# Mikata-Project/adcraft

Hardware: AMD Instinct MI355X
Metric: env-steps/sec (envs×keywords auctions/s) (higher is better)
Workload: dtype i32 cents + f32 (Philox4x32-7 u32); 1 GPU; cfg2: 4096 envs x 256 keywords per GPU, IMPLICIT keywords, mean_volume 128, cvr 0.8, no_vol_prob 0.0, drift False, budget non-binding, 60-step episodes with auto-reset; envs_per_gpu=4096, keywords=256, parallelism=env-sharded x1, collective=none (single GPU), weak_scaling_reference=also.cfg4.value of the N=1 --full line (same per-GPU shard as the N>1 runs)

## Files before the change

adcraft_amd/csrc/adc_law.h:

```cpp
#pragma once
#include <stdint.h>

#if defined(__HIPCC__)
#include <hip/hip_runtime.h>
#define ADC_HD __host__ __device__ __forceinline__
#else
#include <math.h>
#define ADC_HD static inline
#endif

namespace adc {

enum Stage : uint32_t { ST_VOL = 0, ST_AUCTION = 1, ST_DRIFT = 2, ST_XPHANTOM = 3, ST_XREV = 4, ST_ACTION = 5, ST_METRIC = 6, ST_CONV = 7, ST_KEYGEN = 8, ST_AGENT = 9,
                        ST_GBIDDERS = 10, ST_GBID = 11, ST_GCLICK = 12, ST_INTERP = 13, ST_MLP = 14 };
constexpr int kTimesteps = 24;
constexpr int kVolumeMax = 1 << 20;
constexpr float kMoneyMaxCents = 1.0e9f;

struct U4 { uint32_t x, y, z, w; };

ADC_HD uint32_t xor3(uint32_t a, uint32_t b, uint32_t c)
{
#if defined(__HIP_DEVICE_COMPILE__)
    return __builtin_amdgcn_bitop3_b32(a, b, c, 0x96);
// ... 557 lines not shown
    if (any_lane(bound_open(t))) return lower_bound_finish(t, target, loc, scale, tab, stage);
    return bound_accepted(t);
}

ADC_HD uint32_t lower_bound_v(int32_t target, float loc, float scale, const LogTableEntry *tab)
{
    int stage;
    return lower_bound_v_staged(target, loc, scale, tab, stage);
}

ADC_HD void lower_bound_pair(int32_t bid_c, float loc, float scale, const LogTableEntry *tab, uint32_t &w_lo, uint32_t &w_hi, int &stage)
{
    const int32_t b_lo = lower_bound_window(1 - bid_c, loc, scale, tab), b_hi = lower_bound_window(bid_c, loc, scale, tab);
    const BoundTrial t_lo = bound_trial(b_lo, 1 - bid_c, loc, scale, tab), t_hi = bound_trial(b_hi, bid_c, loc, scale, tab);
    w_lo = bound_accepted(t_lo);
    w_hi = bound_accepted(t_hi);
    stage = kBoundAccepted;
    if (any_lane(bound_open(t_lo) || bound_open(t_hi))) {
        int s_lo = kBoundAccepted, s_hi = kBoundAccepted;
        w_lo = lower_bound_finish(t_lo, 1 - bid_c, loc, scale, tab, s_lo);
        w_hi = lower_bound_finish(t_hi, bid_c, loc, scale, tab, s_hi);
        stage = s_lo > s_hi ? s_lo : s_hi;
    }
}

ADC_HD uint64_t offset_reaching_f64(uint32_t W, uint32_t m, uint64_t range)
{
    if (W == 0u) return 0ull;
    if (W > 0x00FFFFFFu || m == 0u) return range;
    const double q = ((double)W * 4294967296.0) / (double)m;
    if (!(q < (double)range)) return range;
    uint64_t d = (uint64_t)q;
    const uint64_t need = (uint64_t)W << 32;
    if (d * m >= need) { if (d > 0ull && (d - 1ull) * m >= need) d -= 1ull; }
    else { d += 1ull; if (d * m < need) d += 1ull; }
    return d < range ? d : range;
}

enum OffsetPath : int { kOffsetCandidate = 0, kOffsetF64 = 1 };

struct OffsetDivisor { uint32_t m; float inv, inv4096; uint64_t m2, m3; };

ADC_HD OffsetDivisor offset_divisor(uint32_t m)
{
    const float inv = fast_rcp((float)m);
    return OffsetDivisor{m, inv, inv * 4096.0f, 2ull * m, 3ull * m};
}

struct OffsetTrial { uint32_t d; bool ok; };

ADC_HD OffsetTrial offset_trial(uint32_t W, const OffsetDivisor &v)
{
    const uint32_t d0 = to_word((float)W * 4294967296.0f * v.inv);
    const uint64_t need = (uint64_t)W << 32;
    const int64_t r0 = (int64_t)(need - (uint64_t)d0 * v.m);
    const uint32_t d1 = d0 + (uint32_t)to_int(__builtin_ceilf((float)(int32_t)(r0 >> 12) * v.inv4096));
    const uint64_t u = need + v.m2 - (uint64_t)d1 * v.m;
    const uint32_t d = d1 - 1u + (u > (uint64_t)v.m ? 1u : 0u) + (u > v.m2 ? 1u : 0u);
    const bool none = W > 0x00FFFFFFu;
    OffsetTrial t;
    t.ok = none | (((u - 1ull) < v.m3) & (v.m >= 0x01000000u));
    t.d = none ? 0xFFFFFFFFu : d;
    return t;
}

ADC_HD uint64_t offset_reaching_staged(uint32_t W, uint32_t m, uint64_t range, int &path)
{
    const OffsetTrial t = offset_trial(W, offset_divisor(m));
    uint64_t d = (W > 0x00FFFFFFu || !((uint64_t)t.d < range)) ? range : (uint64_t)t.d;
    path = kOffsetCandidate;
    if (any_lane(!t.ok)) {
        if (!t.ok) { d = offset_reaching_f64(W, m, range); path = kOffsetF64; }
    }
    return d;
}

ADC_HD uint64_t offset_reaching(uint32_t W, uint32_t m, uint64_t range)
{
    int path;
    return offset_reaching_staged(W, m, range, path);
}

struct WinIntervals { uint32_t c_lo, c_w, n_lo, n_w; };

template <bool F64 = false>
ADC_HD WinIntervals win_intervals_of_bounds(uint32_t w_lo, uint32_t w_hi, uint64_t t_click, const AuctionLaw &law, int *path = nullptr)
{
    WinIntervals r{0u, 0u, 0u, 0u};
    if (path) *path = F64 ? kOffsetF64 : kOffsetCandidate;
    if (!(w_lo < w_hi)) return r;
    const uint64_t top = 0xFFFFFFFFull;
    const uint64_t range_n = 4294967296ull - t_click;
    if constexpr (F64) {
        uint64_t a = offset_reaching_f64(w_lo, law.m_click, t_click), b = offset_reaching_f64(w_hi, law.m_click, t_click);
        b = b < top ? b : top;
        if (a < b) { r.c_lo = (uint32_t)a; r.c_w = (uint32_t)(b - a); }
        a = t_click + offset_reaching_f64(w_lo, law.m_noclick, range_n);
        b = t_click + offset_reaching_f64(w_hi, law.m_noclick, range_n);
        b = b < top ? b : top;
        if (a < b) { r.n_lo = (uint32_t)a; r.n_w = (uint32_t)(b - a); }
    } else {
        const OffsetDivisor vc = offset_divisor(law.m_click), vn = offset_divisor(law.m_noclick);
        const OffsetTrial ta = offset_trial(w_lo, vc), tb = offset_trial(w_hi, vc), tan = offset_trial(w_lo, vn), tbn = offset_trial(w_hi, vn);
        const uint32_t t32 = t_click < top ? (uint32_t)t_click : 0xFFFFFFFFu;
        uint32_t a = ta.d < t32 ? ta.d : t32, b = tb.d < t32 ? tb.d : t32, an = sat_add(t32, tan.d), bn = sat_add(t32, tbn.d);
        const bool all_ok = ta.ok & tb.ok & tan.ok & tbn.ok;
        if (any_lane(!all_ok)) {
#pragma unroll 1
            for (int i = 0; i < 4; ++i) {
                const bool click = i < 2, lower = (i & 1) == 0;
                if (!(i == 0 ? ta.ok : i == 1 ? tb.ok : i == 2 ? tan.ok : tbn.ok)) {
                    uint64_t d = offset_reaching_f64(lower ? w_lo : w_hi, click ? law.m_click : law.m_noclick, click ? t_click : range_n);
                    d += click ? 0ull : t_click;
                    const uint32_t d32 = d < top ? (uint32_t)d : 0xFFFFFFFFu;
                    a = i == 0 ? d32 : a;
                    b = i == 1 ? d32 : b;
                    an = i == 2 ? d32 : an;
                    bn = i == 3 ? d32 : bn;
                }
            }
            if (path && !all_ok) *path = kOffsetF64;
        }
        if (a < b) { r.c_lo = a; r.c_w = b - a; }
        if (an < bn) { r.n_lo = an; r.n_w = bn - an; }
    }
    return r;
}

template <bool SIDE_BY_SIDE = true, bool OFFSETS_F64 = false>
ADC_HD WinIntervals win_intervals(int32_t bid_c, float loc, float scale, uint64_t t_click, const AuctionLaw &law, const LogTableEntry *tab)
{
    uint32_t w_lo, w_hi;
    if constexpr (SIDE_BY_SIDE) {
        int stage;
        lower_bound_pair(bid_c, loc, scale, tab, w_lo, w_hi, stage);
    } else {
        w_lo = lower_bound_v(1 - bid_c, loc, scale, tab);
        w_hi = lower_bound_v(bid_c, loc, scale, tab);
    }
    return win_intervals_of_bounds<OFFSETS_F64>(w_lo, w_hi, t_click, law);
}

struct WinBrackets { WinIntervals out, in; };
constexpr float kWordSlack = 4096.0f;

ADC_HD uint32_t sat_sub(uint32_t a, uint32_t b)
{
#if defined(__clang__)
    return __builtin_elementwise_sub_sat(a, b);
#else
    return a > b ? a - b : 0u;
#endif
}
ADC_HD void lower_bound_estimate(float x_t, float loc, float inv_s, float &est, float &slack)
{
    const float z_t = (x_t - loc) * inv_s;
    const float e_t = __builtin_fabsf(z_t);
    const float mag = min_num(fast_exp2(fma32(e_t, -1.44269504f, 23.0f)), 8388607.0f);
    est = z_t < 0.0f ? mag : 16777215.0f - mag;
    const float rel = fma32(1.0e-6f, fma32(__builtin_fabsf(x_t) + __builtin_fabsf(loc), inv_s, e_t), 2.0e-5f);
    slack = min_num(fma32(mag, rel, 16.0f), 33554432.0f);
}

ADC_HD WinBrackets win_brackets(int32_t bid_c, float loc, float scale, float t_f)
{
    const float inv_s = fast_rcp(__builtin_fabsf(scale));
// ... 351 lines not shown
```

adcraft_amd/csrc/adc_shims.cpp:

```cpp
#include <algorithm>
#include <cmath>
#include <cstdint>
#include <thread>
#include <vector>

#include "../../include/adcraft_engine.h"
#include "adc_law.h"
#include "adc_fast_schedule.h"
#include "adc_interp.h"
#include "adc_mlp.h"
#include "adc_es.h"
#include "adc_pg.h"
#include "adc_pg_kl.h"
#include "adc_pg_shuffle.h"
#include "adc_imitation.h"
#include "adc_td3.h"
#include "adc_sac.h"
#include "adc_pbt.h"
#include "adc_norm.h"
#include "adc_rew_norm.h"
#include "adc_td3_norm.h"
#include "adc_sac_norm.h"
#include "adc_per.h"

// ... 160 lines not shown
    const adc::LogTableEntry *table = host_log_table();
    shim_parallel_for(n, [=](int64_t i0, int64_t i1) {
        for (int64_t i = i0; i < i1; ++i) {
            bool whole = false;
            v_out[i] = adc::lower_bound_v_bisect(target[i], loc[i], scale[i], table, &whole);
            if (whole_range_out) whole_range_out[i] = whole ? 1 : 0;
        }
    });
    return ADC_OK;
}

ADC_EXPORT int adc_win_intervals_host(int64_t n, const int32_t *bid_c, const float *cost_loc, const float *cost_scale, const float *buyside_ctr,
                                      int32_t bisect, uint32_t *out4, uint8_t *stage_out)
{
    if (n < 0 || (n > 0 && (!bid_c || !cost_loc || !cost_scale || !buyside_ctr || !out4))) return ADC_EINVAL;
    const adc::LogTableEntry *table = host_log_table();
    shim_parallel_for(n, [=](int64_t i0, int64_t i1) {
        for (int64_t i = i0; i < i1; ++i) {
            const adc::AuctionLaw law = adc::make_auction_law(buyside_ctr[i]);
            const uint64_t t_click = adc::bernoulli_threshold(buyside_ctr[i]);
            uint32_t w_lo, w_hi;
            int stage = 0;
            if (bisect) {
                bool a = false, b = false;
                w_lo = adc::lower_bound_v_bisect(1 - bid_c[i], cost_loc[i], cost_scale[i], table, &a);
                w_hi = adc::lower_bound_v_bisect(bid_c[i], cost_loc[i], cost_scale[i], table, &b);
                stage = (a || b) ? 1 : 0;
            } else {
                adc::lower_bound_pair(bid_c[i], cost_loc[i], cost_scale[i], table, w_lo, w_hi, stage);
            }
            const adc::WinIntervals r = adc::win_intervals_of_bounds(w_lo, w_hi, t_click, law);
            uint32_t *o = out4 + 4 * i;
            o[0] = r.c_lo; o[1] = r.c_w; o[2] = r.n_lo; o[3] = r.n_w;
            if (stage_out) stage_out[i] = (uint8_t)stage;
        }
    });
    return ADC_OK;
}

ADC_EXPORT int adc_offset_reaching_host(int64_t n, const uint32_t *W, const uint32_t *m, const uint64_t *range, uint64_t *d_out, uint8_t *path_out)
{
    if (n < 0 || (n > 0 && (!W || !m || !range || !d_out))) return ADC_EINVAL;
    shim_parallel_for(n, [=](int64_t i0, int64_t i1) {
        for (int64_t i = i0; i < i1; ++i) {
            int path = 0;
            d_out[i] = adc::offset_reaching_staged(W[i], m[i], range[i], path);
            if (path_out) path_out[i] = (uint8_t)path;
        }
    });
    return ADC_OK;
}

ADC_EXPORT int adc_offset_reaching_f64_host(int64_t n, const uint32_t *W, const uint32_t *m, const uint64_t *range, uint64_t *d_out, uint8_t *path_out)
{
    if (n < 0 || (n > 0 && (!W || !m || !range || !d_out))) return ADC_EINVAL;
    shim_parallel_for(n, [=](int64_t i0, int64_t i1) {
        for (int64_t i = i0; i < i1; ++i) {
            d_out[i] = adc::offset_reaching_f64(W[i], m[i], range[i]);
            if (path_out)
                path_out[i] = W[i] == 0u ? 0 : (W[i] > 0x00FFFFFFu || m[i] == 0u) ? 1
                              : !(((double)W[i] * 4294967296.0) / (double)m[i] < (double)range[i]) ? 2 : 3;
        }
    });
    return ADC_OK;
}

ADC_EXPORT int adc_win_intervals_offsets_host(int64_t n, const int32_t *bid_c, const float *cost_loc, const float *cost_scale, const float *buyside_ctr,
                                              int32_t f64, uint32_t *out4, uint8_t *path_out)
{
    if (n < 0 || (n > 0 && (!bid_c || !cost_loc || !cost_scale || !buyside_ctr || !out4))) return ADC_EINVAL;
    const adc::LogTableEntry *table = host_log_table();
    shim_parallel_for(n, [=](int64_t i0, int64_t i1) {
        for (int64_t i = i0; i < i1; ++i) {
            const adc::AuctionLaw law = adc::make_auction_law(buyside_ctr[i]);
            const uint64_t t_click = adc::bernoulli_threshold(buyside_ctr[i]);
            uint32_t w_lo, w_hi;
            int stage = 0, path = 0;
            adc::lower_bound_pair(bid_c[i], cost_loc[i], cost_scale[i], table, w_lo, w_hi, stage);
            const adc::WinIntervals r = f64 ? adc::win_intervals_of_bounds<true>(w_lo, w_hi, t_click, law, &path)
                                            : adc::win_intervals_of_bounds<false>(w_lo, w_hi, t_click, law, &path);
            uint32_t *o = out4 + 4 * i;
            o[0] = r.c_lo; o[1] = r.c_w; o[2] = r.n_lo; o[3] = r.n_w;
            if (path_out) path_out[i] = (uint8_t)path;
        }
    });
    return ADC_OK;
}

ADC_EXPORT int adc_draw_folded_host(int64_t n, const uint64_t *key, const uint32_t *index, const uint32_t *stage, const uint32_t *keyword,
                                    const uint32_t *tick, uint32_t *plain4, uint32_t *folded4, uint32_t *kw4)
{
    if (n < 0 || (n > 0 && (!key || !index || !stage || !keyword || !tick || !plain4 || !folded4 || !kw4))) return ADC_EINVAL;
    shim_parallel_for(n, [=](int64_t i0, int64_t i1) {
        for (int64_t i = i0; i < i1; ++i) {
            const uint32_t tick_k1 = adc::philox_fold_tick(key[i], tick[i]);
            const adc::U4 a = adc::draw(key[i], index[i], stage[i], keyword[i], tick[i]);
            const adc::U4 b = adc::draw_folded(key[i], index[i], stage[i], keyword[i], tick_k1);
            const adc::U4 c = adc::draw_kw_folded(key[i], index[i], adc::philox_kw_half(stage[i], keyword[i], (uint32_t)key[i]), tick_k1);
            uint32_t *pa = plain4 + 4 * i, *pb = folded4 + 4 * i, *pc = kw4 + 4 * i;
            pa[0] = a.x; pa[1] = a.y; pa[2] = a.z; pa[3] = a.w;
            pb[0] = b.x; pb[1] = b.y; pb[2] = b.z; pb[3] = b.w;
            pc[0] = c.x; pc[1] = c.y; pc[2] = c.z; pc[3] = c.w;
        }
    });
    return ADC_OK;
}

ADC_EXPORT int64_t adc_proven_win_price_host(int64_t n, const int32_t *bid_c, const float *cost_loc, const float *cost_scale, const float *buyside_ctr,
                                             int64_t exhaustive_below, int32_t ends, int32_t samples, uint64_t seed, int64_t *checked, int64_t *first_bad3)
{
    if (n < 0 || (n > 0 && (!bid_c || !cost_loc || !cost_scale || !buyside_ctr)) || ends < 0 || samples < 0) return -1;
    const adc::LogTableEntry *table = host_log_table();
    int64_t bad = 0, count = 0, first[3] = {-1, -1, -1};
    uint64_t s = seed | 1ull;
    auto next = [&]() { s ^= s << 13; s ^= s >> 7; s ^= s << 17; return s; };
    for (int64_t i = 0; i < n; ++i) {
        const float loc = cost_loc[i], scale = cost_scale[i];
        auto check = [&](uint32_t v, int route) {
            ++count;
            if (adc::competitor_cents_of_proven_win(v, loc, scale, table) != adc::competitor_cents_from_v(v, loc, scale, table)) {
                if (first[0] < 0) { first[0] = i; first[1] = (int64_t)v; first[2] = route; }
                ++bad;
            }
        };
        uint32_t w_lo, w_hi;
        int stage = 0;
        adc::lower_bound_pair(bid_c[i], loc, scale, table, w_lo, w_hi, stage);
        if (w_lo < w_hi) {
            const uint32_t width = w_hi - w_lo;
            if ((int64_t)width <= exhaustive_below) {
                for (uint32_t v = w_lo; v < w_hi; ++v) check(v, 0);
            } else {
                for (uint32_t e = 0; e < (uint32_t)ends && e < width; ++e) { check(w_lo + e, 0); check(w_hi - 1u - e, 0); }
                for (int32_t k = 0; k < samples; ++k) check(w_lo + (uint32_t)(next() % width), 0);
            }
        }
        const adc::AuctionLaw law = adc::make_auction_law(buyside_ctr[i]);
        const adc::WinIntervals iv = adc::win_intervals_of_bounds(w_lo, w_hi, adc::bernoulli_threshold(buyside_ctr[i]), law);
        if (iv.c_w != 0u) {
            for (int e = 0; e < 2; ++e) {
                const uint32_t word = e == 0 ? iv.c_lo : iv.c_lo + iv.c_w - 1u;
                const uint32_t v = adc::mulhi32(word, law.m_click);
                check(v < 0x00FFFFFFu ? v : 0x00FFFFFFu, 1);
            }
        }
    }
    if (checked) *checked = count;
    if (first_bad3) { first_bad3[0] = first[0]; first_bad3[1] = first[1]; first_bad3[2] = first[2]; }
    return bad;
}

ADC_EXPORT int64_t adc_fast_schedule_host(const int32_t *vol_k, int32_t tile_kw, int32_t tile_index, int32_t *slots7, int64_t cap, int64_t *totals2,
                                          int32_t *info2)
{
    constexpr int B = adc::kFastTileLanes, WL = adc::kFastWaveLanes, NW = adc::kFastTileWaves;
    if (!vol_k || tile_kw < 1 || tile_kw > B || tile_index < 0 || cap < 0 || (cap > 0 && !slots7)) return ADC_EINVAL;
    int V[B];
    int64_t volume = 0, needed = 0;
    int live = 0;
    for (int t = 0; t < B; ++t) {
        V[t] = t < tile_kw ? vol_k[t] : 0;
        if (V[t] < 0 || V[t] > adc::kVolumeMax) return ADC_EINVAL;
        volume += V[t];
        live += V[t] > 0;
        needed += adc::fast_calls_needed(V[t]);
    }
// ... 1553 lines not shown
```

adcraft_amd/csrc/parts/kernel_fast.inc:

```
constexpr int kQueueCap = 128;
constexpr int kDenseVolumePerKeyword = adc::kDenseVolumePerKeyword;
static_assert(kFastBlock == adc::kFastTileLanes && kWave == adc::kFastWaveLanes, "adc_fast_schedule.h describes this workgroup");

struct alignas(16) KwLawA {
    unsigned int m_click, t_conv;
    float loc, scale;
};
struct alignas(16) KwLawB {
    float mu, sd;
    union {
        struct {
            unsigned int t_click;
            int bid_c;
        } d;
        adc::KwHalf conv;
    };
};
union alignas(16) KwWin {
    adc::WinIntervals iv;
    struct { unsigned int m_noclick, pad0, pad1, pad2; } d;
};

constexpr int kClkShift = 21, kConvShift = 42;
constexpr int kVolBits = 21;
// ... 71 lines not shown
        r.key = v.key[env];
        r.tick = v.tick[env];
        r.drift = v.drift_on && v.drift_pending[env];
        const int hint = v.exact_hint[env];
        r.skip = (hint & ~4) == 2;
        r.emit = LISTS && hint == 1 && v.click_rec != nullptr;
        if (tid < tile_kw && k < v.K && !r.skip) {
            r.vol_mean = param_at(v, ADC_P_VOL_MEAN, env, k);
            r.vol_std = param_at(v, ADC_P_VOL_STD, env, k);
            r.bctr = param_at(v, ADC_P_BCTR, env, k);
            r.sctr = param_at(v, ADC_P_SCTR, env, k);
            r.loc = param_at(v, ADC_P_A, env, k);
            r.scale = param_at(v, ADC_P_B, env, k);
            r.mu = param_at(v, ADC_P_REV_MEAN, env, k);
            r.sd = param_at(v, ADC_P_REV_STD, env, k);
            r.bid = bids[(size_t)env * v.K + k];
        }
        return r;
    };

    const int n_tiles = v.N * tiles;
    const int tile_first = blockIdx.x * tiles_per_wg, tile_last = min(tile_first + tiles_per_wg, n_tiles);
    sh.logtab[tid] = g_log_table[tid];
    for (int i = tid; i <= adc::kNormTableEntries; i += kFastBlock) sh.normtab[i] = g_norm_nodes[i];
    FastRaw next = load_tile(tile_first);

  for (int tile_index = tile_first; tile_index < tile_last; ++tile_index) {
    const FastRaw raw = next;
    if (tile_index + 1 < tile_last) next = load_tile(tile_index + 1);
    if (raw.skip) continue;
    const int env = tile_index / tiles;
    const int tile = tile_index - env * tiles;
    const int k = tile * tile_kw + tid;
    const bool valid = tid < tile_kw && k < v.K;
    const uint64_t key = ((uint64_t)(uint32_t)__builtin_amdgcn_readfirstlane((int)(uint32_t)(raw.key >> 32)) << 32) |
                         (uint32_t)__builtin_amdgcn_readfirstlane((int)(uint32_t)raw.key);
    const uint32_t tick = (uint32_t)__builtin_amdgcn_readfirstlane((int)raw.tick);
    uint32_t tick_k1 = adc::philox_fold_tick(key, tick);
    asm volatile("" : "+s"(tick_k1));
    const uint32_t kw_base = (uint32_t)(tile * tile_kw);
    if (LISTS && raw.emit && tid == 0) v.click_tick[env] = tick + 1u;
    if constexpr (LISTS) { if (raw.emit && !NARROW && tid < adc::kTimesteps) ls.row_count[tid] = 0u; }
    [[maybe_unused]] const unsigned long long t_start = FDBG_T();

    if (tid < (tile_kw + 3) / 4) {
        const adc::U4 w = adc::draw(key, 0u, adc::ST_VOL, (kw_base >> 2) + (uint32_t)tid, tick);
        *reinterpret_cast<uint4 *>(&sh.volw[4 * tid]) = make_uint4(w.x, w.y, w.z, w.w);
    }
    float vol_mean = raw.vol_mean, bctr = raw.bctr, sctr = raw.sctr;
    const float vol_std = raw.vol_std, loc = raw.loc, scale = raw.scale, mu = raw.mu, sd = raw.sd, bid = raw.bid;
    if (valid && raw.drift && drift_keyword(v, env, key, tick - 1u, k, vol_mean, vol_std, bctr, sctr)) {
        param_at(v, ADC_P_VOL_MEAN, env, k) = vol_mean;
        param_at(v, ADC_P_BCTR, env, k) = bctr;
        param_at(v, ADC_P_SCTR, env, k) = sctr;
    }
    sh.a_cnt[tid] = sh.a_cost[tid] = sh.a_rev[tid] = 0ull;
    __syncthreads();
    int V = 0;
    if (valid) {
        float x = adc::fma32(vol_std, normal_tab_nodes(sh.volw[tid], sh.normtab), vol_mean);
        x = x > 0.0f ? x : 0.0f;
        x = x < (float)adc::kVolumeMax ? x : (float)adc::kVolumeMax;
        const float t = __builtin_truncf(x);
        V = (int)t + ((x - t) >= 0.5f ? 1 : 0);
    }
    if constexpr (LISTS) {
        if (raw.emit) {
            const int rows = (int)v.click_row_hint[env], s = V / adc::kTimesteps;
            ls.jcut[tid] = rows >= adc::kTimesteps - 1 ? 0x7FFFFFFF : V - (adc::kTimesteps - 1) * s + rows * s;
            if (tid == 0) ls.price_cut = v.click_price_hint[env];
        }
    }
    {
        const int vsum = wave_sum_i32(V);
        const int live = (int)__popcll(__builtin_amdgcn_ballot_w64(V > 0));
        if (lane == 0) { sh.wave_vol[wv] = vsum; sh.wave_live[wv] = live; }
    }
    __syncthreads();
    int tile_volume = 0, tile_live = 0;
#pragma unroll
    for (int i = 0; i < kFastBlock / kWave; ++i) { tile_volume += sh.wave_vol[i]; tile_live += sh.wave_live[i]; }
    const bool dense = adc::fast_tile_dense(tile_volume, tile_live);
    const int chunk_shift = adc::fast_chunk_shift(tile_volume);
    const int nch = adc::fast_full_items(V, chunk_shift);
    const int ntc = adc::fast_tail_calls(V, chunk_shift);
    const int incl = wave_scan_i32(adc::fast_pack_counts(nch, ntc));
    if (lane == 63) sh.wave_tot[wv] = incl;
    FSLOT_ADD(1, (unsigned long long)adc::fast_calls_needed(V));
    [[maybe_unused]] const unsigned long long t_law = FDBG_T();
    if (V > 0) {
        const uint64_t t_click = adc::bernoulli_threshold(bctr);
        const adc::AuctionLaw law = adc::make_auction_law(bctr);
        const int bid_c = (int)adc::bid_to_cents(bid);
        sh.law_a[tid] = KwLawA{law.m_click, adc::saturate_threshold(adc::bernoulli_threshold(sctr)), loc, scale};
        KwLawB lb;
        lb.mu = mu;
        lb.sd = sd;
        if (dense) {
            lb.conv = adc::philox_kw_half(adc::ST_CONV, kw_base + (uint32_t)tid, (uint32_t)key);
            sh.win[tid].iv = adc::win_intervals(bid_c, loc, scale, t_click, law, sh.logtab);
        } else {
            lb.d.t_click = law.t32;
            lb.d.bid_c = bid_c;
            sh.win[tid].d.m_noclick = law.m_noclick;
        }
        sh.law_b[tid] = lb;
    }
    FDBG_ADD(1, FDBG_T() - t_law);
    __syncthreads();
    int wave_base = 0, total = 0, wave_base2 = 0, total2 = 0;
#pragma unroll
    for (int i = 0; i < kFastBlock / kWave; ++i) {
        const int t = sh.wave_tot[i];
        if (i < wv) { wave_base += adc::fast_packed_items(t); wave_base2 += adc::fast_packed_calls(t); }
        total += adc::fast_packed_items(t);
        total2 += adc::fast_packed_calls(t);
    }
    __syncthreads();
    sh.off[tid] = wave_base + adc::fast_packed_items(incl) - nch;
    {
        const int first_call = wave_base2 + adc::fast_packed_calls(incl) - ntc;
        sh.vol[tid] = V | (first_call << kVolBits);
#pragma unroll
        for (int c = 0; c < adc::kFastTailCallsMax; ++c)
            if (c < ntc) sh.tail_kw[first_call + c] = (unsigned char)tid;
    }
    if (tid == 0) sh.off[kFastBlock] = total;
    __syncthreads();
    [[maybe_unused]] const unsigned long long t_p2 = FDBG_T();
    FDBG_ADD(0, t_p2 - t_start);

    const int wq = __builtin_amdgcn_readfirstlane(wv);
    unsigned int *const qtag = sh.queue.tag[wq];
    unsigned int *const qword = sh.queue.word[wq];
    unsigned int qtail = 0;

    auto resolve_click = [&](bool direct) {
        const uint2 ent = make_uint2(qtag[lane], qword[lane]);
        const unsigned int uu = ent.x >> 24;
        unsigned int acc_off = uu * (unsigned int)sizeof(unsigned long long);
        asm volatile("" : "+v"(acc_off));
        unsigned long long *const acc = (unsigned long long *)((char *)sh.a_cnt + acc_off);
        static_assert(sizeof(KwLawA) == 2 * sizeof(unsigned long long) && sizeof(KwLawB) == sizeof(KwLawA), "law records at twice the accumulators' stride");
        unsigned int law_off;
        asm volatile("v_add_u32 %0, %1, %1" : "=v"(law_off) : "v"(acc_off));
        const KwLawA ka = *(const KwLawA *)((const char *)sh.law_a + law_off);
        const KwLawB kb = *(const KwLawB *)((const char *)sh.law_b + law_off);
        unsigned int price = ent.y;
        if (!direct) {
            unsigned int vv = adc::mulhi32(ent.y, ka.m_click);
            vv = vv < 0x00FFFFFFu ? vv : 0x00FFFFFFu;
            price = (unsigned int)adc::competitor_cents_of_proven_win(vv, ka.loc, ka.scale, sh.logtab);
        }
        const adc::U4 w2 = direct ? adc::draw_folded(key, ent.x & 0x00FFFFFFu, adc::ST_CONV, kw_base + uu, tick_k1)
                                  : adc::draw_kw_folded(key, ent.x & 0x00FFFFFFu, kb.conv, tick_k1);
        const bool conv = adc::bernoulli32(w2.x, ka.t_conv);
        unsigned long long cnt = 1ull << kClkShift;
        if (conv) {
            float x = adc::fma32(kb.sd, normal_tab_nodes(w2.y, sh.normtab), kb.mu);
            x = x > 0.01f ? x : 0.01f;
            atomicAdd(acc + 2 * kFastBlock, (unsigned long long)(unsigned int)adc::money_to_cents(x));
            cnt |= 1ull << kConvShift;
        }
        atomicAdd(acc, cnt);
        atomicAdd(acc + kFastBlock, (unsigned long long)price);
        if constexpr (LISTS) { if (raw.emit) {
            const int j = (int)(ent.x & 0x00FFFFFFu);
            if (j < ls.jcut[uu] || price <= ls.price_cut) {
                const int V = sh.vol[uu] & kVolMask;
                const int s = V / adc::kTimesteps, first = V - (adc::kTimesteps - 1) * s;
                int row = 0, jc = j;
                if (j >= first) {
                    const int d = j - first;
                    int q = (int)((float)d * __builtin_amdgcn_rcpf((float)s));
                    q -= q * s > d ? 1 : 0;
                    q += (q + 1) * s <= d ? 1 : 0;
                    row = 1 + q;
                    jc = d - q * s;
                }
                const unsigned int slot = NARROW ? atomicAdd(&v.click_count[(size_t)env * adc::kTimesteps + row], 1u) : atomicAdd(&ls.row_count[row], 1u);
                if (slot < click_seg_cap(v, row))
                    v.click_rec[click_seg_offset(v, env, row) + slot] = make_uint2(((kw_base + uu) << 20) | (unsigned int)jc, price);
            }
        } }
    };
    auto drain = [&](bool direct) {
        if (qtail >= (unsigned int)kWave) {
            [[maybe_unused]] const unsigned long long tb = FDBG_T();
            __builtin_amdgcn_fence(__ATOMIC_ACQ_REL, "wavefront");
            __builtin_amdgcn_wave_barrier();
            resolve_click(direct);
            qtail -= kWave;
            if ((unsigned int)lane < qtail) { qtag[lane] = qtag[kWave + lane]; qword[lane] = qword[kWave + lane]; }
            FDBG_ADD(4, FDBG_T() - tb);
            FDBG_ADD(7, 1);
        }
    };
    auto push = [&](bool click, unsigned int tagj, unsigned int payload) {
        const unsigned long long m = __builtin_amdgcn_ballot_w64(click);
        const unsigned int rank = __builtin_amdgcn_mbcnt_hi((unsigned int)(m >> 32), __builtin_amdgcn_mbcnt_lo((unsigned int)m, 0u));
        if (click) { (qtag + qtail)[rank] = tagj; (qword + qtail)[rank] = payload; }
        qtail += __popcll(m);
    };
    auto run_item = [&](auto tail_tag, int u, int j0, int n, int calls4) {
        constexpr bool TAIL = decltype(tail_tag)::value;
        const uint32_t kw = kw_base + (uint32_t)u;
        const unsigned int tagj0 = ((unsigned int)u << 24) | (unsigned int)j0;
        const uint32_t call0 = (uint32_t)j0 >> adc::kFastCallShift;
        unsigned int imp = 0;
        if (dense) {
            adc::WinIntervals iv = sh.win[u].iv;
            if (n == 0) iv.c_w = iv.n_w = 0u;
            asm volatile("" : "+v"(iv.c_w), "+v"(iv.n_w));
            uint32_t call = call0;
            for (int i = 0; i < calls4; i += 4, call += 1u) {
                if (TAIL && __builtin_amdgcn_ballot_w64(i < n) == 0ull) break;
                FSLOT_ADD(0, 1ull);
                asm volatile("" : "+v"(call));
                const adc::U4 w = adc::draw_folded(key, call, adc::ST_AUCTION, kw, tick_k1);
#pragma unroll
                for (int h = 0; h < 4; ++h) {
                    const uint32_t word = h == 0 ? w.x : h == 1 ? w.y : h == 2 ? w.z : w.w;
                    bool cw = (word - iv.c_lo) < iv.c_w;
                    bool nw = (word - iv.n_lo) < iv.n_w;
                    if (TAIL) { const bool active = i + h < n; cw = cw && active; nw = nw && active; }
                    add_lane_bit(imp, __builtin_amdgcn_ballot_w64(cw) | __builtin_amdgcn_ballot_w64(nw));
                    push(cw, tagj0 + (unsigned int)(i + h), word);
                    drain(false);
                }
            }
        }
        if (!dense) {
            const KwLawA ka = sh.law_a[u];
            const KwLawB kb = sh.law_b[u];
            const adc::AuctionLaw law{kb.d.t_click, ka.m_click, sh.win[u].d.m_noclick};
            const int bid_c = n > 0 ? kb.d.bid_c : 0;
            uint32_t call = call0;
            for (int i = 0; i < calls4; i += 4, call += 1u) {
                if (TAIL && __builtin_amdgcn_ballot_w64(i < n) == 0ull) break;
                FSLOT_ADD(0, 1ull);
                asm volatile("" : "+v"(call));
                const adc::U4 w = adc::draw_folded(key, call, adc::ST_AUCTION, kw, tick_k1);
#pragma unroll
                for (int h = 0; h < 4; ++h) {
                    const uint32_t word = h == 0 ? w.x : h == 1 ? w.y : h == 2 ? w.z : w.w;
                    bool click_bit;
                    const int comp = adc::auction_outcome_unless_top_word(word, law, ka.loc, ka.scale, sh.logtab, click_bit);
                    bool win = adc::auction_wins(word, bid_c, comp);
                    if (TAIL) win = win && i + h < n;
                    imp += (unsigned int)win;
                    push(win && click_bit, tagj0 + (unsigned int)(i + h), (unsigned int)comp);
                    drain(true);
                }
            }
        }
        if (imp) atomicAdd(&sh.a_cnt[u], (unsigned long long)imp);
    };

#pragma nounroll
    for (int pass = 0; pass < 2; ++pass) {
        const int shift = pass == 0 ? chunk_shift : adc::kFastCallShift;
        const int ptotal = pass == 0 ? total : total2;
        const int part = adc::fast_wave_part(wq, tile_index);
        const int rounds = __builtin_amdgcn_readfirstlane(adc::fast_wave_rounds(ptotal, part));
        const int base = __builtin_amdgcn_readfirstlane(adc::fast_wave_base(ptotal, part));
        if (rounds == 0) continue;
        const int first = adc::fast_lane_first(base, rounds, lane, ptotal);
        int u = 0, u_end = 0;
        if (pass == 0) {
#pragma unroll
            for (int s = kFastBlock / 2; s > 0; s >>= 1)
                if (sh.off[u + s] <= first) u += s;
            u_end = sh.off[u + 1];
        }
        for (int r = 0; r < rounds; ++r) {
            const int item = first + r;
            const bool has = adc::fast_item_exists(item, ptotal);
            [[maybe_unused]] const unsigned long long t_item = FDBG_T();
            int j0 = 0;
            if (pass == 0) {
                while (has && item >= u_end) { u += 1; u_end = sh.off[u + 1]; }
                if (has) j0 = (item - sh.off[u]) << shift;
            } else if (has) {
                u = sh.tail_kw[item];
                const int vw = sh.vol[u];
                j0 = adc::fast_tail_first(vw & kVolMask, chunk_shift) + ((item - (int)((unsigned int)vw >> kVolBits)) << shift);
            }
            FDBG_ADD(2, FDBG_T() - t_item);
            run_item(std::false_type{}, u, j0, has ? 1 << shift : 0, 1 << shift);
        }
    }
    if (__syncthreads_or(adc::fast_partial_count(V) != 0)) {
        const int Vt = sh.vol[tid] & kVolMask;
        run_item(std::true_type{}, tid, adc::fast_partial_first(Vt), adc::fast_partial_count(Vt), 1 << adc::kFastCallShift);
    }
    __builtin_amdgcn_fence(__ATOMIC_ACQ_REL, "wavefront");
    __builtin_amdgcn_wave_barrier();
    if ((unsigned int)lane < qtail) resolve_click(!dense);
    [[maybe_unused]] const unsigned long long t_p3 = FDBG_T();
    FDBG_ADD(3, t_p3 - t_p2);
    __syncthreads();

    if constexpr (LISTS) { if (raw.emit && !NARROW && tid < adc::kTimesteps) v.click_count[(size_t)env * adc::kTimesteps + tid] = ls.row_count[tid]; }
    if (valid) {
        const size_t o = (size_t)env * v.K + k;
        const unsigned long long cnt = sh.a_cnt[tid];
        const long long my_cost = (long long)sh.a_cost[tid];
        const long long r = (long long)sh.a_rev[tid];
        const unsigned int cnt_lo = (unsigned int)cnt, cnt_hi = (unsigned int)(cnt >> 32);
        v.imp[o] = (int)(cnt_lo & 0x1FFFFFu);
        v.clk[o] = (int)(((cnt_lo >> 21) | (cnt_hi << 11)) & 0x1FFFFFu);
        v.conv[o] = (int)(cnt_hi >> 10);
        v.cost[o] = adc::cents_to_dollars_f32(my_cost);
        v.rev[o] = adc::cents_to_dollars_f32(r);
        if (v.metrics_on) metric_add(v, o, r - my_cost);
    }
    if (wv == 0) {
        long long c = 0, p = 0;
#pragma unroll
        for (int i = 0; i < kFastBlock / kWave; ++i) {
            const int u = lane + i * kWave;
            if (u < tile_kw && tile * tile_kw + u < v.K) {
                const long long cc = (long long)sh.a_cost[u];
                c += cc;
                p += (long long)sh.a_rev[u] - cc;
            }
        }
        c = wave_sum_i64(c);
        p = wave_sum_i64(p);
        if (lane == 0) {
            if (tiles == 1) { v.env_cost[env] = c; v.env_profit[env] = p; }
            else {
                atomicAdd((unsigned long long *)&v.env_cost[env], (unsigned long long)c);
                atomicAdd((unsigned long long *)&v.env_profit[env], (unsigned long long)p);
            }
        }
    }
    FDBG_ADD(5, FDBG_T() - t_p3);
    FDBG_ADD(6, 1);
    __syncthreads();
  }
#ifdef ADC_EXP_TIMING
    if (tid == 0) for (int i = 0; i < 8; ++i) atomicAdd(&g_fdbg[blockIdx.x & 255][i], fdbg[i]);
    {
        const unsigned long long needed = (unsigned long long)wave_sum_i64((long long)fslots[1]);
        if (lane == 0) { atomicAdd(&g_fslots[blockIdx.x & 255][0], fslots[0]); atomicAdd(&g_fslots[blockIdx.x & 255][1], needed); }
    }
#endif
}

__device__ __forceinline__ void step_tail(const View &v, int env, uint32_t tick, bool implicit, long long profit_c, double reward_d)
{
    double reward, cum;
    if (implicit) {
        const long long cc = v.cum_cents[env] + profit_c;
        v.cum_cents[env] = cc;
        reward = (double)profit_c / 100.0;
        cum = (double)cc / 100.0;
    } else {
        reward = reward_d;
        cum = v.cum[env] + reward;
        v.cum[env] = cum;
    }
    const bool truncated = cum < -v.loss_threshold;
    const int day = v.day[env] + 1;
    const bool terminated = day >= v.max_days;
    v.reward[env] = reward;
    v.cum_profit[env] = cum;
    v.day_out[env] = day;
    v.term[env] = terminated;
    v.trunc[env] = truncated;
    v.day[env] = day;
    v.tick[env] = tick + 1u;
    if (v.drift_on) v.drift_pending[env] = 1;
    if (v.auto_reset && (terminated || truncated)) {
        v.day[env] = 0; v.cum_cents[env] = 0; v.cum[env] = 0.0;
    }
    v.env_cost[env] = 0;
    v.env_profit[env] = 0;
    if (v.metrics_on) {
        const long long pc = implicit ? profit_c : (long long)__double2ll_rn(reward * 100.0);
        v.metric_env[env] += pc;
        v.metric_env[(size_t)v.NP + env] += 1;
        if (terminated || truncated) v.metric_env[2 * (size_t)v.NP + env] += 1;
        if (truncated) v.metric_env[3 * (size_t)v.NP + env] += 1;
    }
}
```

include/adcraft_engine.h:

```cpp
#ifndef ADCRAFT_ENGINE_H
#define ADCRAFT_ENGINE_H

#include <stddef.h>
#include <stdint.h>

#ifdef __cplusplus
extern "C" {
#endif

#define ADC_ABI_VERSION 5
#define ADC_STREAM_REVISION 5

typedef enum adc_status {
    ADC_OK = 0,
    ADC_EINVAL = -1,
    ADC_EHIP = -2,
    ADC_ENOMEM = -3,
    ADC_ESTATE = -4,
    ADC_ETYPE = -5,
    ADC_ERCCL = -6
} adc_status;

typedef enum adc_model {
    ADC_MODEL_IMPLICIT = 0,
// ... 644 lines not shown
    double rew_min_std;
    int64_t rew_count_cap;
    float rew_clip;
} adc_sac_norm_config;
int adc_sac_norm_config_check(const adc_sac_norm_config *cfg, const char **message);
int adc_engine_sac_norm_init(adc_engine *e, const adc_sac_norm_config *cfg);
int adc_engine_sac_norm_update(adc_engine *e, int64_t *samples);
int adc_engine_sac_norm_state_get(adc_engine *e, int32_t member, int64_t *obs_count, double *obs_mean_d, double *obs_m2_d, float *shift_d, float *scale_d,
                                  int64_t *rew_count, double *rew_mean, double *rew_m2, float *rew_scale);
int adc_engine_sac_norm_state_set(adc_engine *e, int32_t member, int64_t obs_count, const double *obs_mean_d, const double *obs_m2_d, const float *shift_d,
                                  const float *scale_d, int64_t rew_count, double rew_mean, double rew_m2, float rew_scale);
int adc_engine_sac_norm_returns_get(adc_engine *e, double *g_n);
int adc_engine_sac_norm_returns_set(adc_engine *e, const double *g_n);
int adc_engine_sac_norm_copy(adc_engine *e, const int32_t *src_of_member_m);
int adc_sac_y_norm_host(const adc_sac_config *sac, int32_t count, const float *r_b, const uint8_t *done_b, const float *q_b, const float *lp_b, float alpha,
                        float scale, float clip, float *y_b);

typedef struct adc_replay_prio_config {
    uint32_t struct_size;
    float alpha;
    float beta;
    float eps;
    float cap;
} adc_replay_prio_config;
int adc_replay_prio_config_check(const adc_replay_prio_config *cfg, const char **message);
int adc_engine_replay_prio_init(adc_engine *e, const adc_replay_prio_config *cfg);
int adc_engine_replay_prio_set_beta(adc_engine *e, float beta);
int adc_engine_replay_prio_info(adc_engine *e, int32_t member, double *total, float *top);
int adc_engine_replay_prio_fetch(adc_engine *e, int32_t member, int64_t slot, int64_t count, float *leaf);
int adc_engine_replay_prio_load(adc_engine *e, int32_t member, int64_t slot, int64_t count, const float *leaf, float top);
int adc_engine_replay_prio_batch(adc_engine *e, int32_t member, int64_t update, int32_t *idx_b, float *weight_b);
int adc_per_tree_host(int64_t capacity, const float *leaf_c, double *nodes, int64_t *counts);
int adc_per_descend_host(int64_t capacity, const float *leaf_c, double m, int64_t *slot);
int adc_per_sample_host(const adc_replay_prio_config *cfg, int64_t capacity, int64_t size, const float *leaf_c, uint64_t seed, int64_t update, int32_t count,
                        int32_t *idx_b, float *weight_b);
int adc_per_priority_host(const adc_replay_prio_config *cfg, int32_t count, const float *d1_b, const float *d2_b, float *pa_b);
int adc_per_leaf_update_host(int64_t capacity, float *leaf_c, float *top, int32_t count, const int32_t *idx_b, const float *pa_b);

int adc_replay_nstep_check(int32_t n, const char **message);
int adc_engine_replay_nstep_init(adc_engine *e, int32_t n);
int adc_engine_replay_nstep_info(adc_engine *e, int32_t *n);
int adc_engine_replay_nstep_fetch(adc_engine *e, int32_t member, int64_t slot, int64_t count, float *gn);
int adc_engine_replay_nstep_load(adc_engine *e, int32_t member, int64_t slot, int64_t count, const float *gn);
int adc_replay_nstep_host(int32_t n, float gamma, int32_t T, int32_t N, int32_t t0, int32_t t1, const float *reward, const uint8_t *term,
                          const uint8_t *trunc, float *R, uint8_t *done, float *gn, int32_t *m);
int adc_td3_y_nstep_host(const adc_td3_config *td3, int32_t count, const float *r_b, const uint8_t *done_b, const float *q_b, const float *gn_b,
                         float scale, float clip, float *y_b);
int adc_sac_y_nstep_host(const adc_sac_config *sac, int32_t count, const float *r_b, const uint8_t *done_b, const float *q_b, const float *lp_b,
                         const float *gn_b, float alpha, float scale, float clip, float *y_b);

int adc_engine_outcomes_replay(adc_engine *e, int32_t env, int32_t steps_back, const float *bids_k, float budget, int64_t capacity,
                               int32_t *keyword, int32_t *timestep, double *cost, double *revenue, int64_t *count, int32_t *share_volume_k);
int adc_engine_outcomes_replay_tape(adc_engine *e, int32_t env, const float *bids_k, float budget, const adc_tape *tape, int64_t capacity,
                                    int32_t *keyword, int32_t *timestep, double *cost, double *revenue, int64_t *count, int32_t *share_volume_k);

int adc_nth_price_auction(int device_id, double bid, const double *other_bids, int32_t n_auctions, int32_t n_bidders,
                          int32_t n, int32_t num_winners, int32_t *impressions, int32_t *placements, double *costs);

double adc_sigmoid(double x, double s, double t);
double adc_clamp(double x, double lo, double hi);
double adc_threshold_sigmoid(double p, double impression_thresh,
                             double impression_bid_intercept, double impression_slope);
double adc_sum_f64(const double *x, int64_t n);
int64_t adc_count_true(const uint8_t *x, int64_t n);
uint64_t adc_nonneg_int_normal(double mean, double std, uint64_t seed, uint64_t counter);
uint64_t adc_binomial(uint64_t n, double p, uint64_t seed, uint64_t counter);
int adc_cost_create(double x, int64_t n, uint64_t seed, uint64_t counter, double *out_n);
int adc_auction_word_intervals(float bid, float cost_loc, float cost_scale, float buyside_ctr, uint32_t *out4);
int adc_auction_word_brackets(float bid, float cost_loc, float cost_scale, float buyside_ctr, uint32_t *out8);
int64_t adc_check_win_brackets(int64_t n, const float *bid, const float *cost_loc, const float *cost_scale, const float *buyside_ctr,
                               const uint32_t *brackets8, int64_t *first_bad, double *ambiguous_words);
int adc_lower_bound_v_host(int64_t n, const int32_t *target_n, const float *loc_n, const float *scale_n, uint32_t *v_n, uint8_t *stage_n);
int adc_lower_bound_v_bisect_host(int64_t n, const int32_t *target_n, const float *loc_n, const float *scale_n, uint32_t *v_n,
                                  uint8_t *whole_range_n);
int adc_win_intervals_host(int64_t n, const int32_t *bid_cents_n, const float *cost_loc_n, const float *cost_scale_n,
                           const float *buyside_ctr_n, int32_t bisect, uint32_t *out4_n, uint8_t *stage_n);
int adc_draw_folded_host(int64_t n, const uint64_t *key_n, const uint32_t *index_n, const uint32_t *stage_n, const uint32_t *keyword_n,
                         const uint32_t *tick_n, uint32_t *plain4_n, uint32_t *folded4_n, uint32_t *kw4_n);
int64_t adc_proven_win_price_host(int64_t n, const int32_t *bid_cents_n, const float *cost_loc_n, const float *cost_scale_n,
                                  const float *buyside_ctr_n, int64_t exhaustive_below, int32_t ends, int32_t samples, uint64_t seed,
                                  int64_t *checked, int64_t *first_bad3);
int64_t adc_fast_schedule_host(const int32_t *vol_k, int32_t tile_kw, int32_t tile_index, int32_t *slots7, int64_t cap, int64_t *totals2,
                               int32_t *info2);
int adc_sample_random_keyword(uint64_t key, uint32_t keyword, uint32_t serial, float *out8);
int adc_explicit_curve_host(uint64_t key, uint32_t tick, int32_t keyword, int32_t n_samples, float impression_thresh, float a, float b,
                            const double *bid_grid, int32_t n_bids, double *ir_out, double *cpc_out, double *z_mid2_out);
int adc_interp_act_host(float ave_rpc, int32_t num_rpc_obs, float ave_sctr, int32_t num_sctr_obs, double max_observed,
                        double profit_acquisition_threshold, double bid_step, const double *allowed_bids, int32_t n_bids,
                        int32_t n_clicks, const uint16_t *clicks_cent, const float *ave_clicks, int32_t n_cpc, const uint16_t *cpc_cent,
                        const double *ave_cpc, double u, double *margin_out, double *cost_out, double *bid_out, int32_t *index_out,
                        double *mass_out);
double adc_interp_key_host(float bid);
int adc_mlp_act_host(const adc_mlp_config *cfg, int32_t num_keywords, const float *obs_d, const float *const *policy_w,
                     const float *const *policy_b, const float *const *value_w, const float *const *value_b, const float *shift_d,
                     const float *scale_d, const float *log_std_a, const float *normals_a, uint64_t agent_key, uint32_t tick,
                     float budget_override, float *mean_a, float *log_std_out_a, float *action_a, float *logp, float *value,
                     float *bids_k, float *budget);
int adc_mlp_stack_row_host(int32_t num_keywords, int32_t frames, const float *frame0_d0, float *hist_hd0, int32_t *last, int32_t *from,
                           int32_t day, int32_t commit, float *row_d);
int adc_es_config_check(const adc_es_config *cfg, const char **message);
int adc_es_noise_host(uint64_t seed, uint32_t pair, uint32_t generation, int64_t p0, int64_t n, float *eps_n);
int adc_es_update_host(const adc_es_config *cfg, uint64_t seed, int32_t members, int64_t n_params, const double *fitness_m, int64_t generation,
                       float *theta_p, float *m_p, float *v_p, float *grad_p);
int adc_pg_config_check(const adc_pg_config *cfg, const char **message);
int adc_pg_gae_host(const adc_pg_config *cfg, int32_t days, int32_t num_envs, const float *reward_tn, const uint8_t *terminated_tn,
                    const uint8_t *truncated_tn, const float *value_tn, const float *bootstrap_n, float *adv_tn, float *ret_tn);
int adc_pg_param_count_host(const adc_mlp_config *mlp, int32_t num_keywords, int64_t *count);
int adc_pg_grad_host(const adc_mlp_config *mlp, int32_t num_keywords, const adc_pg_config *cfg, const float *theta_q, int64_t count,
                     const float *obs_sd, const float *action_sa, const float *logp_old_s, const float *adv_s, const float *ret_s,
                     const float *value_old_s, float *grad_q, double *sums10, adc_pg_stats *stats);
int adc_pg_step_host(const adc_pg_config *cfg, int64_t n_params, int64_t steps_taken, const float *grad_q, float *theta_q, float *m_q,
                     float *v_q);
int adc_pg_kl_grad_host(const adc_mlp_config *mlp, int32_t num_keywords, const adc_pg_config *cfg, const float *theta_q, int64_t count,
                        const float *obs_sd, const float *action_sa, const float *logp_old_s, const float *adv_s, const float *ret_s,
                        const float *value_old_s, const adc_pg_kl_config *kl, float kl_coef, const float *mean_old_sa, const float *ls_old,
                        int32_t ls_old_per_sample, float *grad_q, double *sums10, double *sums_kl2, adc_pg_stats *stats,
                        adc_pg_kl_stats *kl_stats);
int adc_pg_kl_adapt_host(const adc_pg_kl_config *kl, float coef, double kl_mean, float *coef_next);
int adc_pg_shuffle_order_host(uint64_t seed, int64_t n_s, uint32_t tick, uint32_t *order_out);
int adc_pg_shuffle_stop_host(double approx_kl, float target_kl, int32_t *stop);
int adc_pg_decide_host(const adc_pg_config *cfg, float target_kl, const double *sums10, int64_t count, int32_t *evaluated, int32_t *stop,
                       int32_t *clip, float *scale);
int adc_td3_config_check(const adc_td3_config *cfg, const char **message);
int adc_td3_param_counts_host(const adc_mlp_config *mlp, int32_t num_keywords, const adc_td3_config *cfg, int64_t *actor_p, int64_t *critic_qc);
int adc_td3_batch_indices_host(uint64_t seed, int64_t update, int64_t size, int32_t count, int32_t *idx_b);
int adc_td3_target_host(const adc_mlp_config *mlp, int32_t num_keywords, const adc_td3_config *cfg, uint64_t seed, int64_t update,
                        const float *theta_target_p, const float *psi_target_q, const float *shift_a, const float *scale_a, int32_t count,
                        const float *x2_bd, const float *r_b, const uint8_t *done_b, float *y_b);
int adc_td3_critic_grad_host(const adc_mlp_config *mlp, int32_t num_keywords, const adc_td3_config *cfg, const float *psi_q,
                             const float *shift_a, const float *scale_a, int32_t count, const float *x_bd, const float *a_ba, const float *y_b,
                             float *grad_q, double *sums6);
int adc_td3_actor_grad_host(const adc_mlp_config *mlp, int32_t num_keywords, const adc_td3_config *cfg, const float *theta_p,
                            const float *psi_q, const float *shift_a, const float *scale_a, int32_t count, const float *x_bd, float *grad_p,
                            double *sums2);
int adc_td3_polyak_host(float tau, int64_t n, const float *param_n, float *target_n);
int adc_sac_config_check(const adc_sac_config *cfg, const char **message);
int adc_sac_param_counts_host(const adc_mlp_config *mlp, int32_t num_keywords, const adc_sac_config *cfg, int64_t *actor_p, int64_t *critic_qc);
int adc_sac_logp_host(const adc_mlp_config *mlp, int32_t num_keywords, float eps_sq, int32_t count, const float *mean_ba, const float *raw_ba,
                      const float *z_ba, float *u_ba, float *t_ba, float *lp_b);
int adc_sac_target_host(const adc_mlp_config *mlp, int32_t num_keywords, const adc_sac_config *cfg, uint64_t seed, int64_t update, float alpha,
                        const float *theta_p, const float *psi_target_q, int32_t count, const float *x2_bd, const float *r_b, const uint8_t *done_b,
                        float *y_b, float *lp_b);
int adc_sac_critic_grad_host(const adc_mlp_config *mlp, int32_t num_keywords, const adc_sac_config *cfg, const float *psi_q, int32_t count,
                             const float *x_bd, const float *u_ba, const float *y_b, float *grad_q, double *sums6);
int adc_sac_actor_grad_host(const adc_mlp_config *mlp, int32_t num_keywords, const adc_sac_config *cfg, uint64_t seed, int64_t update, float alpha,
                            const float *theta_p, const float *psi_q, int32_t count, const float *x_bd, float *grad_p, float *lp_b, double *sums4);
int adc_sac_alpha_step_host(const adc_sac_config *cfg, int64_t steps_taken, double lp_sum, int32_t count, float *la3, float *alpha);
float adc_sac_log_alpha_init_host(float init_alpha);
int adc_pbt_fitness_host(int32_t days, int32_t num_envs, int32_t members, const float *reward_tn, double *fitness_m);
int adc_pbt_plan_host(const adc_pbt_config *cfg, uint64_t seed, int32_t members, int64_t round, const double *fitness_m, double *smoothed_m,
                      int32_t *rank_m, int32_t *src_m, uint32_t *bits_m);
int adc_pbt_explore_host(const adc_pbt_config *cfg, int32_t kind, uint32_t bits, const float *donor_hp8, const float *own_hp8, float *out_hp8);
int adc_mlp_config_check(const adc_mlp_config *cfg, int32_t num_keywords, const char **message);
float adc_mlp_math_host(int32_t fn, float x);
int adc_mlp_squash_host(int32_t count, const float *u_a, const float *lo_a, const float *hi_a, float *out_a);
int64_t adc_mlp_math_sweep_host(int32_t fn, float lo, float hi, double *out3, int64_t *violations4);
uint64_t adc_mlp_agent_key_host(uint64_t seed);
uint64_t adc_mlp_default_agent_key_host(uint64_t engine_seed, uint64_t global_env_id);
int adc_debug_philox_device(int device_id, int64_t n, const uint32_t *ctr4, const uint32_t *key2, uint32_t *out4);
int adc_debug_chain_device(int device_id, double r0, int64_t n, const double *x, double *out2);
int adc_debug_walk_stats(adc_engine *e, int64_t stats[4], int reset);
int adc_debug_direct_days(adc_engine *e, int64_t *env_days, int reset);
int adc_debug_win_brackets_device(int device_id, int64_t n, const float *bid, const float *cost_loc, const float *cost_scale,
                                  const float *buyside_ctr, uint32_t *out8);

#ifdef __cplusplus
// ... 4 lines not shown
```

Before: 6.850 billion keyword-steps/s.

## Skip dead keywords, push queue via inline LDS asm, count impressions from clicks

In the dense path, keywords whose win intervals are both empty are marked dead and given zero work volume, so no chunks or tail calls are scheduled for them. The click queue push now uses inline ds_write2st64_b32 with an explicit exec mask and a byte-address cursor instead of two separate LDS stores. Impression counting keeps only non-click wins and adds clicks back at writeback, removing one ballot per word. The tail item's block-wide __syncthreads_or becomes a per-wave ballot. A host shim is added to check dead-keyword detection against exhaustive auctions. The inline asm depends on the LDS queue layout, and skipping dead keywords assumes the intervals are exact.

```diff
diff --git a/adcraft_amd/csrc/adc_law.h b/adcraft_amd/csrc/adc_law.h
--- a/adcraft_amd/csrc/adc_law.h
+++ b/adcraft_amd/csrc/adc_law.h
@@ -663,6 +663,8 @@
 }
 
 struct WinIntervals { uint32_t c_lo, c_w, n_lo, n_w; };
+
+ADC_HD bool fast_keyword_is_dead(const WinIntervals &iv) { return iv.c_w == 0u && iv.n_w == 0u; }
 
 template <bool F64 = false>
 ADC_HD WinIntervals win_intervals_of_bounds(uint32_t w_lo, uint32_t w_hi, uint64_t t_click, const AuctionLaw &law, int *path = nullptr)
diff --git a/adcraft_amd/csrc/adc_shims.cpp b/adcraft_amd/csrc/adc_shims.cpp
--- a/adcraft_amd/csrc/adc_shims.cpp
+++ b/adcraft_amd/csrc/adc_shims.cpp
@@ -266,6 +266,47 @@
             uint32_t *o = out4 + 4 * i;
             o[0] = r.c_lo; o[1] = r.c_w; o[2] = r.n_lo; o[3] = r.n_w;
             if (path_out) path_out[i] = (uint8_t)path;
+        }
+    });
+    return ADC_OK;
+}
+
+ADC_EXPORT int adc_fast_dead_keywords_host(int64_t n, const float *bid, const float *cost_loc, const float *cost_scale, const float *buyside_ctr,
+                                           int32_t n_random, uint64_t seed, uint8_t *dead_out, uint32_t *out4, int64_t *wins2)
+{
+    if (n < 0 || n_random < 0 || (n > 0 && (!bid || !cost_loc || !cost_scale || !buyside_ctr || !dead_out))) return ADC_EINVAL;
+    const adc::LogTableEntry *table = host_log_table();
+    shim_parallel_for(n, [=](int64_t i0, int64_t i1) {
+        for (int64_t i = i0; i < i1; ++i) {
+            const int32_t bid_c = (int32_t)adc::bid_to_cents(bid[i]);
+            const adc::AuctionLaw law = adc::make_auction_law(buyside_ctr[i]);
+            const uint64_t t_click = adc::bernoulli_threshold(buyside_ctr[i]);
+            const adc::WinIntervals iv = adc::win_intervals(bid_c, cost_loc[i], cost_scale[i], t_click, law, table);
+            dead_out[i] = adc::fast_keyword_is_dead(iv) ? 1 : 0;
+            if (out4) { uint32_t *o = out4 + 4 * i; o[0] = iv.c_lo; o[1] = iv.c_w; o[2] = iv.n_lo; o[3] = iv.n_w; }
+            if (!wins2) continue;
+            int64_t by_auction = 0, by_interval = 0;
+            auto word = [&](uint32_t w) {
+                bool click;
+                const int32_t comp = adc::auction_outcome(w, law, cost_loc[i], cost_scale[i], table, click);
+                by_auction += adc::auction_wins(w, bid_c, comp) ? 1 : 0;
+                by_interval += ((w - iv.c_lo) < iv.c_w || (w - iv.n_lo) < iv.n_w) ? 1 : 0;
+            };
+            const uint64_t top = 0xFFFFFFFEull;
+            word(0u);
+            word((uint32_t)(t_click == 0 ? 0ull : t_click - 1 < top ? t_click - 1 : top));
+            word((uint32_t)(t_click < top ? t_click : top));
+            word((uint32_t)top);
+            uint64_t s = seed + 0x9E3779B97F4A7C15ull * (uint64_t)(i + 1);
+            for (int32_t r = 0; r < n_random; ++r) {
+                s += 0x9E3779B97F4A7C15ull;
+                uint64_t z = s;
+                z = (z ^ (z >> 30)) * 0xBF58476D1CE4E5B9ull;
+                z = (z ^ (z >> 27)) * 0x94D049BB133111EBull;
+                word((uint32_t)((z ^ (z >> 31)) >> 32));
+            }
+            wins2[2 * i] = by_auction;
+            wins2[2 * i + 1] = by_interval;
         }
     });
     return ADC_OK;
diff --git a/adcraft_amd/csrc/parts/kernel_fast.inc b/adcraft_amd/csrc/parts/kernel_fast.inc
--- a/adcraft_amd/csrc/parts/kernel_fast.inc
+++ b/adcraft_amd/csrc/parts/kernel_fast.inc
@@ -177,12 +177,8 @@
     for (int i = 0; i < kFastBlock / kWave; ++i) { tile_volume += sh.wave_vol[i]; tile_live += sh.wave_live[i]; }
     const bool dense = adc::fast_tile_dense(tile_volume, tile_live);
     const int chunk_shift = adc::fast_chunk_shift(tile_volume);
-    const int nch = adc::fast_full_items(V, chunk_shift);
-    const int ntc = adc::fast_tail_calls(V, chunk_shift);
-    const int incl = wave_scan_i32(adc::fast_pack_counts(nch, ntc));
-    if (lane == 63) sh.wave_tot[wv] = incl;
-    FSLOT_ADD(1, (unsigned long long)adc::fast_calls_needed(V));
     [[maybe_unused]] const unsigned long long t_law = FDBG_T();
+    bool dead = false;
     if (V > 0) {
         const uint64_t t_click = adc::bernoulli_threshold(bctr);
         const adc::AuctionLaw law = adc::make_auction_law(bctr);
@@ -193,7 +189,9 @@
         lb.sd = sd;
         if (dense) {
             lb.conv = adc::philox_kw_half(adc::ST_CONV, kw_base + (uint32_t)tid, (uint32_t)key);
-            sh.win[tid].iv = adc::win_intervals(bid_c, loc, scale, t_click, law, sh.logtab);
+            const adc::WinIntervals iv = adc::win_intervals(bid_c, loc, scale, t_click, law, sh.logtab);
+            sh.win[tid].iv = iv;
+            dead = adc::fast_keyword_is_dead(iv);
         } else {
             lb.d.t_click = law.t32;
             lb.d.bid_c = bid_c;
@@ -202,6 +200,12 @@
         sh.law_b[tid] = lb;
     }
     FDBG_ADD(1, FDBG_T() - t_law);
+    const int Vw = dead ? 0 : V;
+    const int nch = adc::fast_full_items(Vw, chunk_shift);
+    const int ntc = adc::fast_tail_calls(Vw, chunk_shift);
+    const int incl = wave_scan_i32(adc::fast_pack_counts(nch, ntc));
+    if (lane == 63) sh.wave_tot[wv] = incl;
+    FSLOT_ADD(1, (unsigned long long)adc::fast_calls_needed(Vw));
     __syncthreads();
     int wave_base = 0, total = 0, wave_base2 = 0, total2 = 0;
 #pragma unroll
@@ -215,7 +219,7 @@
     sh.off[tid] = wave_base + adc::fast_packed_items(incl) - nch;
     {
         const int first_call = wave_base2 + adc::fast_packed_calls(incl) - ntc;
-        sh.vol[tid] = V | (first_call << kVolBits);
+        sh.vol[tid] = Vw | (first_call << kVolBits);
 #pragma unroll
         for (int c = 0; c < adc::kFastTailCallsMax; ++c)
             if (c < ntc) sh.tail_kw[first_call + c] = (unsigned char)tid;
@@ -227,8 +231,12 @@
 
     const int wq = __builtin_amdgcn_readfirstlane(wv);
     unsigned int *const qtag = sh.queue.tag[wq];
-    unsigned int *const qword = sh.queue.word[wq];
-    unsigned int qtail = 0;
+    unsigned int *const qword = qtag + sizeof(sh.queue.tag) / sizeof(unsigned int);
+    typedef __attribute__((address_space(3))) unsigned int LdsWord;
+    const unsigned int qbase = (unsigned int)__builtin_amdgcn_readfirstlane((int)(unsigned int)(size_t)(LdsWord *)qtag);
+    constexpr unsigned int kBatchBytes = kWave * sizeof(unsigned int);
+    static_assert(sizeof(sh.queue.tag) == 8 * 64 * sizeof(unsigned int), "a push writes the word at offset1:8 of ds_write2st64_b32");
+    unsigned int qaddr = qbase;
 
     auto resolve_click = [&](bool direct) {
         const uint2 ent = make_uint2(qtag[lane], qword[lane]);
@@ -280,22 +288,23 @@
         } }
     };
     auto drain = [&](bool direct) {
-        if (qtail >= (unsigned int)kWave) {
+        if (qaddr >= qbase + kBatchBytes) {
             [[maybe_unused]] const unsigned long long tb = FDBG_T();
             __builtin_amdgcn_fence(__ATOMIC_ACQ_REL, "wavefront");
             __builtin_amdgcn_wave_barrier();
             resolve_click(direct);
-            qtail -= kWave;
-            if ((unsigned int)lane < qtail) { qtag[lane] = qtag[kWave + lane]; qword[lane] = qword[kWave + lane]; }
+            qaddr -= kBatchBytes;
+            if ((unsigned int)lane < (qaddr - qbase) / (unsigned int)sizeof(unsigned int)) { qtag[lane] = qtag[kWave + lane]; qword[lane] = qword[kWave + lane]; }
             FDBG_ADD(4, FDBG_T() - tb);
             FDBG_ADD(7, 1);
         }
     };
-    auto push = [&](bool click, unsigned int tagj, unsigned int payload) {
-        const unsigned long long m = __builtin_amdgcn_ballot_w64(click);
+    auto push = [&](unsigned long long m, unsigned int tagj, unsigned int payload) {
         const unsigned int rank = __builtin_amdgcn_mbcnt_hi((unsigned int)(m >> 32), __builtin_amdgcn_mbcnt_lo((unsigned int)m, 0u));
-        if (click) { (qtag + qtail)[rank] = tagj; (qword + qtail)[rank] = payload; }
-        qtail += __popcll(m);
+        const unsigned int slot = rank * (unsigned int)sizeof(unsigned int) + qaddr;
+        asm volatile("s_mov_b64 exec, %0\n\tds_write2st64_b32 %1, %2, %3 offset1:8\n\ts_mov_b64 exec, -1"
+                     :: "s"(m), "v"(slot), "v"(tagj), "v"(payload) : "memory");
+        qaddr += (unsigned int)__popcll(m) * (unsigned int)sizeof(unsigned int);
     };
     auto run_item = [&](auto tail_tag, int u, int j0, int n, int calls4) {
         constexpr bool TAIL = decltype(tail_tag)::value;
@@ -319,8 +328,8 @@
                     bool cw = (word - iv.c_lo) < iv.c_w;
                     bool nw = (word - iv.n_lo) < iv.n_w;
                     if (TAIL) { const bool active = i + h < n; cw = cw && active; nw = nw && active; }
-                    add_lane_bit(imp, __builtin_amdgcn_ballot_w64(cw) | __builtin_amdgcn_ballot_w64(nw));
-                    push(cw, tagj0 + (unsigned int)(i + h), word);
+                    add_lane_bit(imp, __builtin_amdgcn_ballot_w64(nw));
+                    push(__builtin_amdgcn_ballot_w64(cw), tagj0 + (unsigned int)(i + h), word);
                     drain(false);
                 }
             }
@@ -343,8 +352,8 @@
                     const int comp = adc::auction_outcome_unless_top_word(word, law, ka.loc, ka.scale, sh.logtab, click_bit);
                     bool win = adc::auction_wins(word, bid_c, comp);
                     if (TAIL) win = win && i + h < n;
-                    imp += (unsigned int)win;
-                    push(win && click_bit, tagj0 + (unsigned int)(i + h), (unsigned int)comp);
+                    imp += (unsigned int)(win && !click_bit);
+                    push(__builtin_amdgcn_ballot_w64(win && click_bit), tagj0 + (unsigned int)(i + h), (unsigned int)comp);
                     drain(true);
                 }
             }
@@ -385,13 +394,14 @@
             run_item(std::false_type{}, u, j0, has ? 1 << shift : 0, 1 << shift);
         }
     }
-    if (__syncthreads_or(adc::fast_partial_count(V) != 0)) {
+    {
         const int Vt = sh.vol[tid] & kVolMask;
-        run_item(std::true_type{}, tid, adc::fast_partial_first(Vt), adc::fast_partial_count(Vt), 1 << adc::kFastCallShift);
+        if (__builtin_amdgcn_ballot_w64(adc::fast_partial_count(Vt) != 0) != 0ull)
+            run_item(std::true_type{}, tid, adc::fast_partial_first(Vt), adc::fast_partial_count(Vt), 1 << adc::kFastCallShift);
     }
     __builtin_amdgcn_fence(__ATOMIC_ACQ_REL, "wavefront");
     __builtin_amdgcn_wave_barrier();
-    if ((unsigned int)lane < qtail) resolve_click(!dense);
+    if ((unsigned int)lane < (qaddr - qbase) / (unsigned int)sizeof(unsigned int)) resolve_click(!dense);
     [[maybe_unused]] const unsigned long long t_p3 = FDBG_T();
     FDBG_ADD(3, t_p3 - t_p2);
     __syncthreads();
@@ -403,8 +413,9 @@
         const long long my_cost = (long long)sh.a_cost[tid];
         const long long r = (long long)sh.a_rev[tid];
         const unsigned int cnt_lo = (unsigned int)cnt, cnt_hi = (unsigned int)(cnt >> 32);
-        v.imp[o] = (int)(cnt_lo & 0x1FFFFFu);
-        v.clk[o] = (int)(((cnt_lo >> 21) | (cnt_hi << 11)) & 0x1FFFFFu);
+        const unsigned int clicks = ((cnt_lo >> 21) | (cnt_hi << 11)) & 0x1FFFFFu;
+        v.imp[o] = (int)((cnt_lo & 0x1FFFFFu) + clicks);
+        v.clk[o] = (int)clicks;
         v.conv[o] = (int)(cnt_hi >> 10);
         v.cost[o] = adc::cents_to_dollars_f32(my_cost);
         v.rev[o] = adc::cents_to_dollars_f32(r);
diff --git a/include/adcraft_engine.h b/include/adcraft_engine.h
--- a/include/adcraft_engine.h
+++ b/include/adcraft_engine.h
@@ -750,6 +750,8 @@
                                   int64_t *checked, int64_t *first_bad3);
 int64_t adc_fast_schedule_host(const int32_t *vol_k, int32_t tile_kw, int32_t tile_index, int32_t *slots7, int64_t cap, int64_t *totals2,
                                int32_t *info2);
+int adc_fast_dead_keywords_host(int64_t n, const float *bid_n, const float *cost_loc_n, const float *cost_scale_n, const float *buyside_ctr_n,
+                                int32_t n_random, uint64_t seed, uint8_t *dead_n, uint32_t *out4_n, int64_t *wins2_n);
 int adc_sample_random_keyword(uint64_t key, uint32_t keyword, uint32_t serial, float *out8);
 int adc_explicit_curve_host(uint64_t key, uint32_t tick, int32_t keyword, int32_t n_samples, float impression_thresh, float a, float b,
                             const double *bid_grid, int32_t n_bids, double *ir_out, double *cpc_out, double *z_mid2_out);
```

New measurement: 7.050 billion keyword-steps/s (median of 6 runs). 1.03x the previous value.
